# Lzcstan/DrugLAMP

Hardware: AMD Instinct MI355X
Metric: drug-protein pairs/sec training step (higher is better)
Workload: dtype bf16; 1 GPU; DrugLAMP training step (cls step, epoch 1; fwd+bwd+grad all-reduce+AdamW), BindingDB-shaped synthetic pairs (512 drug nodes/tokens, 2304 protein tokens = 256 sites, pre-extracted 384-d/640-d LLM embeddings), global batch 256 = 256 per GPU x 1; per_gpu_batch=256, global_batch=256, parallelism=dp1, step_kind=cls, epoch=1, hip_graph=False, protein_seq_len=2304, distinct_batches=8, first_touch_steps=8, padding_rows=computed once, protein_cnn_rows=distinct rows, streams=independent branches on side HIP streams

## Files before the change

druglamp_amd/_lib.py:

```python
from __future__ import annotations

import ctypes as C
import os

import torch

_HERE = os.path.dirname(os.path.abspath(__file__))
_variant = os.environ.get("DL_USE_STUDY_LIB", "")
if _variant and not _variant.endswith(".so"):
    raise RuntimeError("DL_USE_STUDY_LIB=%s: the -DDL_STUDY build (libdruglamp_hip_study.so) was removed; commit 97fb613 is the last "
                       "that builds it (python -m druglamp_amd.build --study).  Only a variant library name (libdruglamp_hip_<variant>.so) "
                       "is accepted." % _variant)
LIB_PATH = os.path.join(_HERE, "lib", _variant or "libdruglamp_hip.so")

DL_F32, DL_BF16 = 0, 1

c_i64, c_i32, c_f32, c_u64, c_vp, c_sz = C.c_int64, C.c_int32, C.c_float, C.c_uint64, C.c_void_p, C.c_size_t


class ReduceItem(C.Structure):
    _fields_ = [
        ("kind", c_i32), ("out_dtype", c_i32),
        ("src", c_vp), ("out", c_vp),
        ("mn", c_i64), ("ldc", c_i64),
        ("N", c_i32), ("splits", c_i32), ("accumulate", c_i32), ("M", c_i32),
        ("cs_slabs", c_vp), ("cs_out", c_vp),
    ]


REDUCE_BATCH_MAX = 24
GEMM_GROUP_MAX = 16


class GemmArgs(C.Structure):
    _fields_ = [
        ("X", c_vp), ("ldx", c_i64), ("x_kslow", c_i32),
        ("W", c_vp), ("ldw", c_i64), ("w_kslow", c_i32),
        ("C", c_vp), ("ldc", c_i64),
        ("M", c_i64), ("N", c_i64), ("K", c_i64),
        ("in_dtype", c_i32), ("out_dtype", c_i32),
        ("bias", c_vp),
        ("residual", c_vp), ("ldr", c_i64),
        ("res_row_mod", c_i64),
        ("res_before_dropout", c_i32),
        ("act", c_i32),
        ("pre_out", c_vp), ("ldp", c_i64),
        ("dact_pre", c_vp), ("lddp", c_i64),
        ("dropout_p", c_f32), ("dropout_seed", c_u64),
        ("accumulate", c_i32),
        ("split_k", c_i32), ("workspace", c_vp), ("workspace_bytes", c_sz),
        ("x_colsum", c_vp),
        ("dropout_seed_offset", c_vp),
        ("algo", c_i32),
        ("tile_tickets", c_vp),
        ("deferred", C.POINTER(ReduceItem)),
        ("prof_tag", c_i32),
    ]


FLAG_PROT_PERIOD, FLAG_DRUG_TOKEN_PAD, FLAG_GCN_NODE_PAD, FLAG_PLAN_ROWS, FLAG_PAIR_INDEX = 1, 2, 4, 8, 16
FLAG_KEY_TABLE = 32
FLAG_MAP_COLS = 64
TAG_OTHER, TAG_QKV_OUT, TAG_FFN, TAG_CONV, TAG_WGRAD, TAG_ADAPTOR = 0, 1, 2, 3, 4, 5
TAG_NAMES = {0: "other", 1: "qkv_out", 2: "ffn", 3: "conv", 4: "wgrad", 5: "adaptor"}


class AttnFwdArgs(C.Structure):
    _fields_ = [
        ("Q", c_vp), ("K", c_vp), ("V", c_vp), ("O", c_vp), ("LSE", c_vp), ("raw_logits", c_vp),
        ("q_ps", c_i64), ("q_hs", c_i64), ("q_rs", c_i64),
        ("k_ps", c_i64), ("k_hs", c_i64), ("k_rs", c_i64),
        ("v_ps", c_i64), ("v_hs", c_i64), ("v_rs", c_i64),
        ("o_ps", c_i64), ("o_hs", c_i64), ("o_rs", c_i64), ("o_ss", c_i64),
        ("n_problems", c_i32), ("n_heads", c_i32), ("n_segments", c_i32), ("partner_shift", c_i32),
        ("Lq", c_i32), ("Lk", c_i32), ("head_dim", c_i32), ("dtype", c_i32),
        ("scale", c_f32),
        ("algo", c_i32),
        ("key_tail_rows", c_i32), ("key_tail_weight", c_f32),
    ]


class AttnBwdArgs(C.Structure):
    _fields_ = [
        ("Q", c_vp), ("K", c_vp), ("V", c_vp), ("O", c_vp), ("dO", c_vp),
        ("LSE", c_vp), ("Delta", c_vp),
        ("dQ", c_vp), ("dK", c_vp), ("dV", c_vp),
        ("q_ps", c_i64), ("q_hs", c_i64), ("q_rs", c_i64),
        ("k_ps", c_i64), ("k_hs", c_i64), ("k_rs", c_i64),
        ("v_ps", c_i64), ("v_hs", c_i64), ("v_rs", c_i64),
        ("o_ps", c_i64), ("o_hs", c_i64), ("o_rs", c_i64), ("o_ss", c_i64),
        ("do_ps", c_i64), ("do_hs", c_i64), ("do_rs", c_i64), ("do_ss", c_i64),
        ("dq_ps", c_i64), ("dq_hs", c_i64), ("dq_rs", c_i64),
        ("dk_ps", c_i64), ("dk_hs", c_i64), ("dk_rs", c_i64),
        ("dv_ps", c_i64), ("dv_hs", c_i64), ("dv_rs", c_i64),
        ("n_problems", c_i32), ("n_heads", c_i32), ("n_segments", c_i32), ("partner_shift", c_i32),
        ("Lq", c_i32), ("Lk", c_i32), ("head_dim", c_i32), ("dtype", c_i32),
        ("scale", c_f32),
        ("algo", c_i32),
        ("key_tail_rows", c_i32), ("key_tail_weight", c_f32),
    ]


class AttnProbsArgs(C.Structure):
    _fields_ = [
        ("Q", c_vp), ("K", c_vp), ("LSE", c_vp), ("out", c_vp), ("out_ld", c_i64),
        ("q_ps", c_i64), ("q_hs", c_i64), ("q_rs", c_i64),
        ("k_ps", c_i64), ("k_hs", c_i64), ("k_rs", c_i64),
        ("n_problems", c_i32), ("n_heads", c_i32), ("n_segments", c_i32), ("partner_shift", c_i32),
        ("Lq", c_i32), ("Lk", c_i32), ("head_dim", c_i32), ("dtype", c_i32),
        ("scale", c_f32),
        ("head_mean", c_i32), ("key_tail_rows", c_i32), ("key_tail_weight", c_f32), ("expand_tail", c_i32),
        ("workspace", c_vp), ("workspace_bytes", c_sz),
    ]


# ... 66 lines not shown
        ("q_index", c_vp), ("kv_index", c_vp), ("kv_row0", c_vp), ("kv_keys", c_vp), ("kv_tail_weight", c_vp), ("flags", c_vp),
        ("q_es", c_i64), ("q_rs", c_i64), ("k_rs", c_i64), ("mass_ps", c_i64), ("site_ps", c_i64), ("kv_total_rows", c_i64),
        ("n_pairs", c_i32), ("n_q", c_i32), ("n_kv", c_i32), ("Lq", c_i32), ("head_dim", c_i32), ("dtype", c_i32),
        ("out_cols", c_i32),
        ("scale", c_f32),
        ("key_tail_rows", c_i32),
        ("reserved", c_i32),
    ]


class PgcaPairsAttrArgs(C.Structure):
    _fields_ = [
        ("Q", c_vp), ("K", c_vp), ("dO", c_vp), ("sites", c_vp), ("d_sites", c_vp), ("key_attr", c_vp), ("site_attr", c_vp),
        ("q_index", c_vp), ("kv_index", c_vp), ("flags", c_vp),
        ("q_es", c_i64), ("q_rs", c_i64), ("k_es", c_i64), ("k_rs", c_i64), ("do_ps", c_i64), ("do_rs", c_i64),
        ("left_es", c_i64), ("left_rs", c_i64), ("dl_ps", c_i64), ("dl_rs", c_i64), ("mass_ps", c_i64), ("site_ps", c_i64),
        ("n_pairs", c_i32), ("n_q", c_i32), ("n_kv", c_i32), ("Lq", c_i32), ("Lk", c_i32), ("head_dim", c_i32), ("dtype", c_i32),
        ("out_cols", c_i32), ("left_cols", c_i32),
        ("scale", c_f32),
        ("key_tail_rows", c_i32), ("key_tail_weight", c_f32),
        ("reserved", c_i32),
    ]


class PgcaPairsRaggedAttrArgs(C.Structure):
    _fields_ = [
        ("Q", c_vp), ("K", c_vp), ("dO", c_vp), ("sites", c_vp), ("d_sites", c_vp), ("key_attr", c_vp), ("site_attr", c_vp),
        ("q_index", c_vp), ("kv_index", c_vp), ("kv_row0", c_vp), ("kv_keys", c_vp), ("kv_tail_weight", c_vp), ("flags", c_vp),
        ("q_es", c_i64), ("q_rs", c_i64), ("k_rs", c_i64), ("do_ps", c_i64), ("do_rs", c_i64),
        ("left_es", c_i64), ("left_rs", c_i64), ("dl_ps", c_i64), ("dl_rs", c_i64), ("mass_ps", c_i64), ("site_ps", c_i64),
        ("kv_total_rows", c_i64),
        ("n_pairs", c_i32), ("n_q", c_i32), ("n_kv", c_i32), ("Lq", c_i32), ("head_dim", c_i32), ("dtype", c_i32),
        ("out_cols", c_i32), ("left_cols", c_i32),
        ("scale", c_f32),
        ("key_tail_rows", c_i32),
        ("reserved", c_i32),
    ]


class NtxentSide(C.Structure):
    _fields_ = [("q", c_vp), ("k", c_vp), ("n", c_i64), ("gid_offset", c_i64), ("lse", c_vp)]


class NtxentArgs(C.Structure):
    _fields_ = [("a", NtxentSide), ("b", NtxentSide), ("n_global", c_i64), ("d", c_i64), ("dtype", c_i32),
                ("temperature", c_f32)]


SIGNATURES = {
    "dl_last_error": (C.c_char_p, []),
    "dl_version": (c_i32, []),
    "dl_gemm_workspace_bytes": (c_sz, [C.POINTER(GemmArgs)]),
    "dl_gemm": (c_i32, [C.POINTER(GemmArgs), c_vp]),
    "dl_gemm_pair": (c_i32, [C.POINTER(GemmArgs), C.POINTER(GemmArgs), c_vp]),
    "dl_gemm_group_plan": (c_i32, [C.POINTER(GemmArgs), c_i32, C.POINTER(c_i32)]),
    "dl_gemm_group": (c_i32, [C.POINTER(GemmArgs), c_i32, c_vp]),
    "dl_reduce_batch": (c_i32, [C.POINTER(ReduceItem), c_i32, c_vp]),
    "dl_colsum": (c_i32, [c_vp, c_i64, c_i64, c_i64, c_i32, c_vp, c_i32, c_vp, c_sz, c_vp]),
    "dl_colsum_workspace_bytes": (c_sz, [c_i64, c_i64]),
    "dl_bn_workspace_bytes": (c_sz, [c_i64, c_i64]),
    "dl_bn_stats": (c_i32, [c_vp, c_i64, c_i64, c_i64, c_i64, c_i64, c_i32, c_vp, c_vp, c_sz, c_vp]),
    "dl_bn_apply_fwd": (c_i32, [c_vp, c_vp, c_vp, c_vp, c_vp, c_vp, c_i64, c_i64, c_i64, c_i64, c_i64, c_i32, c_vp]),
    "dl_bn_bwd_reduce": (c_i32, [c_vp, c_vp, c_vp, c_vp, c_i64, c_i64, c_i64, c_i64, c_i64, c_i32, c_vp, c_vp, c_sz, c_vp]),
    "dl_bn_tail_fix": (c_i32, [c_vp, c_vp, c_vp, c_vp, c_vp, c_vp, c_f32, c_i32, c_i64, c_i64, c_i64, c_i64, c_i32, c_vp]),
    "dl_bn_apply_relu_fwd": (c_i32, [c_vp, c_vp, c_vp, c_vp, c_vp, c_vp, c_i64, c_i64, c_i32, c_vp]),
    "dl_bn_relu_bwd": (c_i32, [c_vp, c_vp, c_vp, c_vp, c_vp, c_vp, c_f32, c_vp, c_vp, c_i64, c_i64, c_i32, c_vp, c_sz, c_vp]),
    "dl_bn_bwd_apply": (c_i32, [c_vp, c_vp, c_vp, c_vp, c_vp, c_vp, c_f32, c_i32, c_vp, c_i64, c_i64, c_i64, c_i64, c_i64,
                                c_i32, c_vp]),
    "dl_layernorm_fwd": (c_i32, [c_vp, c_i64, c_vp, c_vp, c_vp, c_i64, c_vp, c_vp, c_i64, c_i64, c_f32, c_i32, c_vp]),
    "dl_layernorm_bwd_workspace_bytes": (c_sz, [c_i64, c_i64]),
    "dl_layernorm_bwd": (c_i32, [c_vp, c_i64, c_i64, c_vp, c_i64, c_vp, c_vp, c_vp, c_vp, c_i64, c_vp, c_i64, c_vp, c_vp,
                                 c_i32, c_i64, c_i64, c_i32, c_vp, c_sz, C.POINTER(ReduceItem), c_vp]),
    "dl_attn_fwd": (c_i32, [C.POINTER(AttnFwdArgs), c_vp]),
    "dl_attn_bwd": (c_i32, [C.POINTER(AttnBwdArgs), c_vp]),
    "dl_attn_probs_workspace_bytes": (c_sz, [C.POINTER(AttnProbsArgs)]),
    "dl_attn_probs": (c_i32, [C.POINTER(AttnProbsArgs), c_vp]),
    "dl_pgca_pairs_fwd": (c_i32, [C.POINTER(PgcaPairsArgs), c_vp]),
    "dl_pgca_pairs_ragged_fwd": (c_i32, [C.POINTER(PgcaPairsRaggedArgs), c_vp]),
    "dl_pgca_pairs_probs": (c_i32, [C.POINTER(PgcaPairsProbsArgs), c_vp]),
    "dl_pgca_pairs_ragged_probs": (c_i32, [C.POINTER(PgcaPairsRaggedProbsArgs), c_vp]),
    "dl_pgca_pairs_profile": (c_i32, [C.POINTER(PgcaPairsProfileArgs), c_vp]),
    "dl_pgca_pairs_ragged_profile": (c_i32, [C.POINTER(PgcaPairsRaggedProfileArgs), c_vp]),
    "dl_pgca_pairs_attr": (c_i32, [C.POINTER(PgcaPairsAttrArgs), c_vp]),
    "dl_pgca_pairs_ragged_attr": (c_i32, [C.POINTER(PgcaPairsRaggedAttrArgs), c_vp]),
    "dl_token_gate_fwd": (c_i32, [c_vp, c_vp, c_vp, c_vp, c_i64, c_i64, c_i64, c_i32, c_i32, c_i32, c_vp]),
    "dl_token_gate_bwd": (c_i32, [c_vp, c_vp, c_vp, c_vp, c_vp, c_i64, c_i64, c_i64, c_i32, c_i32, c_i32, c_vp]),
    "dl_gate_dpre": (c_i32, [c_vp, c_vp, c_vp, c_vp, c_i64, c_i64, c_i32, c_i32, c_vp]),
    "dl_add_rowmod_dropout": (c_i32, [c_vp, c_vp, c_vp, c_i64, c_i64, c_i64, c_f32, c_u64, c_vp, c_i32, c_vp]),
    "dl_dropout_apply": (c_i32, [c_vp, c_vp, c_i64, c_i64, c_i64, c_i64, c_f32, c_u64, c_vp, c_i32, c_vp]),
    "dl_fill_pool": (c_i32, [c_vp, c_vp, c_vp, c_i64, c_i64, c_i64, c_i32, c_i32, c_i32, c_vp]),
    "dl_cnn_sitepool_fwd": (c_i32, [c_vp, c_vp, c_i64, c_i64, c_i64, c_i32, c_i32, c_i32, c_vp]),
    "dl_cnn_sitepool_bwd": (c_i32, [c_vp, c_vp, c_i64, c_i64, c_i64, c_i32, c_i32, c_i32, c_vp]),
    "dl_bn_stats_finalize": (c_i32, [c_vp, c_i64, c_i64, c_i64, c_i64, c_i64, c_vp, c_i32, c_i64, c_f32, c_f32, c_vp, c_vp, c_vp, c_vp, c_vp, c_vp, c_vp, c_sz, c_vp]),
    "dl_bn_finalize": (c_i32, [c_vp, c_i64, c_f32, c_f32, c_vp, c_vp, c_vp, c_vp, c_vp, c_i64, c_vp]),
    "dl_interleave_streams": (c_i32, [c_vp, c_vp, c_i64, c_i64, c_i32, c_i32, c_vp]),
    "dl_norm_adjacency": (c_i32, [c_vp, c_vp, c_i64, c_i32, c_i32, c_vp]),
    "dl_graph_aggregate": (c_i32, [c_vp, c_vp, c_vp, c_i64, c_i32, c_i32, c_i32, c_i32, c_i32, c_vp]),
    "dl_concat2": (c_i32, [c_vp, c_vp, c_vp, c_i64, c_i64, c_i64, c_i32, c_vp]),
    "dl_gather_pad": (c_i32, [c_vp, c_vp, c_vp, c_vp, c_i64, c_i64, c_i64, c_i32, c_i32, c_vp]),
    "dl_embed_pad": (c_i32, [c_vp, c_vp, c_vp, c_vp, c_i64, c_i64, c_i32, c_i32, c_i32, c_i32, c_vp]),
    "dl_weight_prep": (c_i32, [c_vp, c_vp, c_i32, c_i32, c_vp]),
    "dl_gelu_bwd": (c_i32, [c_vp, c_vp, c_vp, c_i64, c_i32, c_vp]),
    "dl_cast": (c_i32, [c_vp, c_i32, c_vp, c_i32, c_i64, c_vp]),
    "dl_rowmod_sum": (c_i32, [c_vp, c_vp, c_i64, c_i64, c_i64, c_i32, c_i32, c_vp]),
    "dl_cos_rowloss_fwd": (c_i32, [c_vp, c_vp, c_vp, c_vp, c_i64, c_i64, c_vp]),
    "dl_cos_rowloss_bwd": (c_i32, [c_vp, c_vp, c_f32, c_vp, c_i64, c_i64, c_vp]),
# ... 128 lines not shown
```

druglamp_amd/csrc/gemm.hip:

```cpp
#include <stdlib.h>
#include <stdint.h>
#include <algorithm>
#include <type_traits>
#include "common.cuh"

namespace {

constexpr int BKB = 128;
constexpr int NTHREADS = 256;

template <typename T, int TW> struct TileGeom {
  static constexpr int BT = 32 * TW;
  static constexpr int BKE = BKB / (int)sizeof(T);
  static constexpr int PITCH_KSLOW = BT * (int)sizeof(T);
  static constexpr int CPR_KSLOW = PITCH_KSLOW / 16;
  static constexpr int TILE_KCONTIG = BT * BKB;
  static constexpr int TILE_KSLOW = BKE * PITCH_KSLOW;
  static constexpr int TILE_BYTES = TILE_KSLOW > TILE_KCONTIG ? TILE_KSLOW : TILE_KCONTIG;
};

struct GemmP {
  const char* X; const char* W; char* C;
  int64_t ldx, ldw, ldc;
  int M, N, K, k_per_split, mt, nt, splits;
// ... 372 lines not shown
        if (full) {
          const f32x4 q0 = load4<T>(src), q1 = load4<T>(src + 4);
#pragma unroll
          for (int r = 0; r < 4; ++r) { resv[r] = q0[r]; resv[4 + r] = q1[r]; }
        } else {
          for (int r = 0; r < nvalid; ++r) resv[r] = to_f32(src[r]);
        }
        if (p.res_before_dropout) {
#pragma unroll
          for (int r = 0; r < 8; ++r) v[r] += resv[r];
        }
      }
      if (p.drop_thr16) {
        f32x4 d0 = {v[0], v[1], v[2], v[3]}, d1 = {v[4], v[5], v[6], v[7]};
        d0 = dl_dropout4(d0, p.seed + seed_off_v, (uint64_t)m, (uint64_t)n, (uint64_t)p.N, p.drop_thr16, p.drop_inv_keep);
        d1 = dl_dropout4(d1, p.seed + seed_off_v, (uint64_t)m, (uint64_t)(n + 4), (uint64_t)p.N, p.drop_thr16, p.drop_inv_keep);
#pragma unroll
        for (int r = 0; r < 4; ++r) { v[r] = d0[r]; v[4 + r] = d1[r]; }
      }
      if (p.res && !p.res_before_dropout) {
#pragma unroll
        for (int r = 0; r < 8; ++r) v[r] += resv[r];
      }
      TO* dst = reinterpret_cast<TO*>(p.C) + (int64_t)m * p.ldc + n;
      if (p.accumulate) {
        if (full) {
          const f32x4 o0 = load4<TO>(dst), o1 = load4<TO>(dst + 4);
#pragma unroll
          for (int r = 0; r < 4; ++r) { v[r] += o0[r]; v[4 + r] += o1[r]; }
        } else {
          for (int r = 0; r < nvalid; ++r) v[r] += to_f32(dst[r]);
        }
      }
      if (full) {
        if constexpr (sizeof(TO) == 2) {
          u32x4 o = {pack_bf16x2(v[0], v[1]), pack_bf16x2(v[2], v[3]), pack_bf16x2(v[4], v[5]), pack_bf16x2(v[6], v[7])};
          *reinterpret_cast<u32x4*>(dst) = o;
        } else {
          *reinterpret_cast<f32x4*>(dst) = f32x4{v[0], v[1], v[2], v[3]};
          *reinterpret_cast<f32x4*>(dst + 4) = f32x4{v[4], v[5], v[6], v[7]};
        }
      } else {
        for (int r = 0; r < nvalid; ++r) dst[r] = from_f32<TO>(v[r]);
      }
    }
  }
  if (!have_next) break;
  it = itn;
  __syncthreads();
  }
}

#include "gemm_big.cuh"

template <typename TO>
__global__ void splitk_reduce_kernel(const float* __restrict__ slabs, TO* __restrict__ out,
                                     int64_t mn, int64_t ldc, int N, int splits, int accumulate,
                                     const float* __restrict__ cs_slabs, float* __restrict__ cs_out, int M, uint32_t main_blocks) {
  if (blockIdx.x >= main_blocks) {
    const int m = (int)(blockIdx.x - main_blocks) * blockDim.x + threadIdx.x;
    if (m < M) {
      float a0 = 0.f, a1 = 0.f;
      int z = 0;
      for (; z + 1 < splits; z += 2) { a0 += cs_slabs[(int64_t)z * M + m]; a1 += cs_slabs[(int64_t)(z + 1) * M + m]; }
      if (z < splits) a0 += cs_slabs[(int64_t)z * M + m];
      cs_out[m] = a0 + a1;
    }
    return;
  }
  const int64_t i4 = ((int64_t)blockIdx.x * blockDim.x + threadIdx.x) * 4;
  if (i4 >= mn) return;
  f32x4 s0 = {0.f, 0.f, 0.f, 0.f}, s1 = s0, s2 = s0, s3 = s0;
  int z = 0;
  for (; z + 3 < splits; z += 4) {
    s0 += *reinterpret_cast<const f32x4*>(slabs + (int64_t)z * mn + i4);
    s1 += *reinterpret_cast<const f32x4*>(slabs + (int64_t)(z + 1) * mn + i4);
    s2 += *reinterpret_cast<const f32x4*>(slabs + (int64_t)(z + 2) * mn + i4);
    s3 += *reinterpret_cast<const f32x4*>(slabs + (int64_t)(z + 3) * mn + i4);
  }
  for (; z < splits; ++z) s0 += *reinterpret_cast<const f32x4*>(slabs + (int64_t)z * mn + i4);
  f32x4 s = (s0 + s1) + (s2 + s3);
  const int64_t m = i4 / N, n = i4 % N;
  TO* dst = out + m * ldc + n;
  if (accumulate) { const f32x4 o = load4<TO>(dst); s += o; }
  store4<TO>(dst, s);
}

int pick_tw(const dl_gemm_args* a) {
  if (a->x_kslow && a->w_kslow && a->split_k >= 0) {
    const int64_t tiles128 = ((a->M + 127) / 128) * ((a->N + 127) / 128);
    if (tiles128 <= 4 && a->M >= 64 && a->N >= 64 && a->K % (BKB / (int)dl_dtype_size(a->in_dtype)) == 0) return 2;
  }
  return 4;
}

int auto_split(int64_t M, int64_t N, int64_t K, int bke, int bt) {
  const int64_t tiles = ((M + bt - 1) / bt) * ((N + bt - 1) / bt);
  if (tiles >= 192) return 1;
  constexpr int round_wgs = 512, max_sp = 256;
  int64_t want = round_wgs / tiles;
  if (want < 1) want = 1;
  int64_t ksteps = (K + bke - 1) / bke;
  int64_t maxs = ksteps / 4;
  if (maxs < 1) maxs = 1;
  if (want > maxs) want = maxs;
  if (want > max_sp) want = max_sp;
  return (int)(want < 1 ? 1 : want);
}

int big_tt_plan(const dl_gemm_args* a, int* bm_out);
static int trim_splits(int64_t K, int step, int sp) {
  const int64_t ksteps = (K + step - 1) / step;
  if (sp > ksteps) sp = (int)ksteps;
  if (sp < 1) sp = 1;
  const int64_t per = (ksteps + sp - 1) / sp;
  return (int)((ksteps + per - 1) / per);
}
int resolve_split(const dl_gemm_args* a) {
  { const int sp = big_tt_plan(a, nullptr); if (sp > 0) return trim_splits(a->K, 64, sp); }
  const int bke = BKB / (int)dl_dtype_size(a->in_dtype);
  if (a->split_k > 0) return trim_splits(a->K, bke, a->split_k);
  if (a->split_k < 0) return 1;
  const bool plain = !a->bias && !a->residual && !a->act && !a->pre_out && !a->dact_pre &&
                     a->dropout_p <= 0.f && a->out_dtype == DL_F32 && (a->N % 4 == 0);
  return plain ? trim_splits(a->K, bke, auto_split(a->M, a->N, a->K, bke, 32 * pick_tw(a))) : 1;
}

int pick_epi(const GemmP& p, bool split) {
  int epi = 1;
  if (!split && (p.N % 8 == 0) && !p.accumulate && p.res_row_mod == 0 && !(p.res && p.res_before_dropout)) {
    const bool drop = p.drop_thr16 != 0;
    if (!p.res && !p.act && !p.pre_out && !p.dact_pre && !drop) epi = 0;
    else if (p.act == 1 && p.pre_out && !p.res && !p.dact_pre) epi = 2;
    else if (p.res && !p.act && !p.pre_out && !p.dact_pre) epi = 3;
    else if (p.dact_pre && !p.res && !p.act && !p.pre_out && !p.bias) epi = 4;
    else if (p.act == 2 && !p.res && !p.pre_out && !p.dact_pre && !drop) epi = 5;
  }
  return epi;
}

bool big_eligible(const dl_gemm_args* a, const GemmP& p, int sp) {
  if (a->algo == DL_GEMM_ALGO_TILE128) return false;
  if (sp > 1 || a->in_dtype != DL_BF16 || a->out_dtype != DL_BF16 || a->x_kslow || a->w_kslow) return false;
  if (pick_epi(p, false) == 1) return false;
  if (a->K % 64 != 0 || a->N <= 128) return false;
  const int64_t tiles = ((a->M + 255) / 256) * ((a->N + 255) / 256);
  return tiles >= 192;
}
constexpr int LAT_MIN_K = 512;
constexpr int LAT_MAX_TILES = 256;
bool lat_eligible(const dl_gemm_args* a, const GemmP& p, int sp) {
  if (a->algo == DL_GEMM_ALGO_TILE128) return false;
  if (sp > 1 || a->in_dtype != DL_BF16 || a->out_dtype != DL_BF16 || a->x_kslow || a->w_kslow) return false;
  if (pick_epi(p, false) == 1) return false;
  if (a->K % 64 != 0 || a->K < LAT_MIN_K || a->N < 128) return false;
  const int64_t tiles = ((a->M + 127) / 128) * ((a->N + 127) / 128);
  return tiles <= LAT_MAX_TILES;
}
template <int XF, int WM, int WN, int RB, int NS>
void launch_big_form(const GemmP& p, hipStream_t s, uint32_t max_wgs, uint32_t threads) {
  const uint32_t ntiles = (uint32_t)p.mt * p.nt;
  const uint32_t nblocks = ntiles < max_wgs ? ntiles : max_wgs;
#define DL_BIG(E) hipLaunchKernelGGL((gemm_big_kernel<XF, WM, WN, RB, NS, E>), dim3(nblocks), dim3(threads), 0, s, p)
  switch (pick_epi(p, false)) {
    case 0: DL_BIG(0); break;
    case 2: DL_BIG(2); break;
    case 3: DL_BIG(3); break;
    case 4: DL_BIG(4); break;
    default: DL_BIG(5); break;
  }
#undef DL_BIG
}
void launch_lat(const GemmP& p, hipStream_t s) { launch_big_form<4, 2, 2, 128, 4>(p, s, 256u, 256u); }
void launch_big(const GemmP& p, hipStream_t s) { launch_big_form<8, 2, 4, 128, 2>(p, s, 256u, 512u); }

int big_tt_plan(const dl_gemm_args* a, int* bm_out) {
  if (a->algo == DL_GEMM_ALGO_TILE128) return 0;
  if (a->in_dtype != DL_BF16 || !a->x_kslow || !a->w_kslow || a->split_k != 0) return 0;
  const bool plain = !a->bias && !a->residual && !a->act && !a->pre_out && !a->dact_pre && a->dropout_p <= 0.f;
  if (!plain || a->M % 8 != 0 || a->N % 8 != 0 || a->N < 192 || a->M < 96 || a->K < 4096) return 0;
  const bool big = a->M > 128 && a->M * a->N >= 640 * 1024;
  const int bm = big ? 256 : 128;
  if (!big) {
    const double work = (double)a->M * (double)a->N * (double)a->K;
    if (a->M > 128 ? work < 1.0e10 : (a->N < 640 || a->K < 262144)) return 0;
  }
  const int64_t tiles = ((a->M + bm - 1) / bm) * ((a->N + 255) / 256);
  if (tiles > 256) return 0;
  int64_t sp = 256 / tiles;
  const int64_t ksteps = (a->K + 63) / 64;
  if (sp > ksteps / 4) sp = ksteps / 4;
  if (sp < 1) sp = 1;
  if (bm_out) *bm_out = bm;
  return (int)sp;
}
template <int XF, int KS, int NS, bool PF>
void launch_big_tt2(const GemmP& p, hipStream_t s, uint32_t nblocks) {
  if (p.cs_slabs) hipLaunchKernelGGL((gemm_big_tt2_kernel<XF, 2, 4, true, KS, NS, PF>), dim3(nblocks), dim3(512), 0, s, p);
  else hipLaunchKernelGGL((gemm_big_tt2_kernel<XF, 2, 4, false, KS, NS, PF>), dim3(nblocks), dim3(512), 0, s, p);
}
void launch_big_tt(const GemmP& p, hipStream_t s, int bm) {
  const uint32_t ntiles = (uint32_t)p.mt * p.nt * p.splits;
  const uint32_t nblocks = ntiles < 256u ? ntiles : 256u;
  if (bm == 256) launch_big_tt2<8, 32, 4, false>(p, s, nblocks); else launch_big_tt2<4, 64, 3, false>(p, s, nblocks);
}

template <typename T, typename TO, bool XS, bool WS, bool SPLIT, bool DMA>
void launch(const GemmP& p, hipStream_t s, int tw) {
  const int epi = pick_epi(p, SPLIT);
  const uint32_t ntiles = (uint32_t)p.mt * p.nt * p.splits;
// ... 20 lines not shown
      case 2: DL_LAUNCH(2); break;
      case 3: DL_LAUNCH(3); break;
      case 4: DL_LAUNCH(4); break;
      case 5: DL_LAUNCH(5); break;
      default: DL_LAUNCH(1); break;
    }
  }
#undef DL_LAUNCH
}

template <typename T, typename TO, bool SPLIT>
int dispatch_layout(const dl_gemm_args* a, const GemmP& p, hipStream_t s, int tw) {
  const int bke = BKB / (int)sizeof(T);
  const bool dma = (a->K % bke == 0) && (p.k_per_split % bke == 0);
  if (!a->x_kslow && !a->w_kslow) { if (dma) launch<T, TO, false, false, SPLIT, true>(p, s, tw); else launch<T, TO, false, false, SPLIT, false>(p, s, tw); }
  else if (!a->x_kslow && a->w_kslow) { if (dma) launch<T, TO, false, true, SPLIT, true>(p, s, tw); else launch<T, TO, false, true, SPLIT, false>(p, s, tw); }
  else if (a->x_kslow && a->w_kslow) { if (dma) launch<T, TO, true, true, SPLIT, true>(p, s, tw); else launch<T, TO, true, true, SPLIT, false>(p, s, tw); }
  else {
    dl_set_error("dl_gemm: layout x_kslow=1,w_kslow=0 is not instantiated");
    return DL_ERR_UNSUPPORTED;
  }
  return DL_OK;
}

}

extern "C" size_t dl_gemm_workspace_bytes(const dl_gemm_args* a) {
  if (!a) return 0;
  const int sp = resolve_split(a);
  const size_t cs = a->x_colsum ? (size_t)sp * (size_t)a->M * sizeof(float) : 0;
  if (big_tt_plan(a, nullptr) > 0 || sp > 1 || a->x_colsum) return (size_t)sp * (size_t)a->M * (size_t)a->N * sizeof(float) + cs;
  return 0;
}

namespace {
static double gemm_algorithmic_bytes(const dl_gemm_args* a) {
  const double es = (double)dl_dtype_size(a->in_dtype), oes = (double)dl_dtype_size(a->out_dtype);
  auto span = [](double rows, double len, double pitch) { return pitch < len ? (rows - 1.0) * pitch + len : rows * len; };
  const double x = a->x_kslow ? span((double)a->K, (double)a->M, (double)a->ldx) : span((double)a->M, (double)a->K, (double)a->ldx);
  const double w = a->w_kslow ? span((double)a->K, (double)a->N, (double)a->ldw) : span((double)a->N, (double)a->K, (double)a->ldw);
  const double mn = (double)a->M * (double)a->N;
  double bytes = (x + w) * es + mn * oes;
  if (a->pre_out) bytes += mn * es;
  if (a->dact_pre) bytes += mn * es;
  if (a->residual) bytes += (a->res_row_mod > 0 ? (double)a->res_row_mod * (double)a->N : mn) * es;
  if (a->accumulate) bytes += mn * oes;
  if (a->bias) bytes += (double)a->N * 4.0;
  return bytes;
}
constexpr int DL_PAIR_FALLBACK = 1;
int gemm_run(const dl_gemm_args* a, const dl_gemm_args* b, dl_stream stream);
}
extern "C" int dl_gemm(const dl_gemm_args* a, dl_stream stream) { return gemm_run(a, nullptr, stream); }

extern "C" int dl_gemm_pair(const dl_gemm_args* a, const dl_gemm_args* b, dl_stream stream) {
  DL_CHECK_ARG(a && b, DL_ERR_ARG, "dl_gemm_pair: null argument block");
  auto same_presence = [](const void* x, const void* y) { return (x == nullptr) == (y == nullptr); };
  const bool twin =
      a->M == b->M && a->N == b->N && a->K == b->K && a->ldx == b->ldx && a->ldw == b->ldw && a->ldc == b->ldc &&
      a->x_kslow == b->x_kslow && a->w_kslow == b->w_kslow && a->in_dtype == b->in_dtype && a->out_dtype == b->out_dtype &&
      a->ldr == b->ldr && a->res_row_mod == b->res_row_mod && a->res_before_dropout == b->res_before_dropout &&
      a->act == b->act && a->ldp == b->ldp && a->lddp == b->lddp && a->dropout_p == b->dropout_p &&
      a->accumulate == b->accumulate && a->split_k == b->split_k && a->algo == b->algo &&
      a->dropout_seed_offset == b->dropout_seed_offset && a->tile_tickets == b->tile_tickets &&
      same_presence(a->bias, b->bias) && same_presence(a->residual, b->residual) && same_presence(a->pre_out, b->pre_out) &&
      same_presence(a->dact_pre, b->dact_pre) && !a->x_colsum && !b->x_colsum && !a->deferred && !b->deferred &&
      (((uintptr_t)b->X | (uintptr_t)b->W | (uintptr_t)b->C | (uintptr_t)b->bias | (uintptr_t)b->residual |
        (uintptr_t)b->pre_out | (uintptr_t)b->dact_pre) & 15) == 0;
  if (twin) {
    const int rc = gemm_run(a, b, stream);
    if (rc != DL_PAIR_FALLBACK) return rc;
  }
  const int rc = gemm_run(a, nullptr, stream);
  return rc != DL_OK ? rc : gemm_run(b, nullptr, stream);
}

namespace {
int gemm_run(const dl_gemm_args* a, const dl_gemm_args* b, dl_stream stream) {
  hipStream_t s = (hipStream_t)stream;
  DL_CHECK_ARG(a && a->X && a->W && a->C, DL_ERR_ARG, "dl_gemm: null operand");
  if (b) DL_CHECK_ARG(b->X && b->W && b->C, DL_ERR_ARG, "dl_gemm_pair: null operand");
  DL_CHECK_ARG(a->M > 0 && a->N > 0 && a->K > 0, DL_ERR_SHAPE, "dl_gemm: bad shape M=%ld N=%ld K=%ld",
               (long)a->M, (long)a->N, (long)a->K);
  DL_CHECK_ARG(a->M < (1ll << 30) && a->N < (1ll << 30) && a->K < (1ll << 30), DL_ERR_SHAPE,
               "dl_gemm: dims must fit int32");
  DL_CHECK_ARG(a->in_dtype == DL_F32 || a->in_dtype == DL_BF16, DL_ERR_ARG, "dl_gemm: bad in_dtype");
  DL_CHECK_ARG(a->out_dtype == DL_F32 || a->out_dtype == a->in_dtype, DL_ERR_ARG,
               "dl_gemm: out_dtype must be f32 or in_dtype");
  const int es = (int)dl_dtype_size(a->in_dtype);
  const int epc = 16 / es;
  DL_CHECK_ARG(a->ldx % epc == 0 && a->ldw % epc == 0, DL_ERR_ALIGN,
               "dl_gemm: ldx/ldw must be multiples of %d elements", epc);
  DL_CHECK_ARG(((uintptr_t)a->X & 15) == 0 && ((uintptr_t)a->W & 15) == 0, DL_ERR_ALIGN,
               "dl_gemm: X/W must be 16-byte aligned");
  if (!a->x_kslow) DL_CHECK_ARG(a->K % epc == 0, DL_ERR_ALIGN, "dl_gemm: K %% %d != 0", epc);
  else DL_CHECK_ARG(a->M % epc == 0, DL_ERR_ALIGN, "dl_gemm: M %% %d != 0 for k-slow X", epc);
  if (!a->w_kslow) DL_CHECK_ARG(a->K % epc == 0, DL_ERR_ALIGN, "dl_gemm: K %% %d != 0", epc);
  else DL_CHECK_ARG(a->N % epc == 0, DL_ERR_ALIGN, "dl_gemm: N %% %d != 0 for k-slow W", epc);
  if (a->N % 8 == 0) {
    DL_CHECK_ARG(a->ldc % 8 == 0 && ((uintptr_t)a->C % 16) == 0, DL_ERR_ALIGN,
                 "dl_gemm: C / ldc not aligned for 16-byte stores (N %% 8 == 0 path)");
    DL_CHECK_ARG(!a->residual || (a->ldr % 8 == 0 && ((uintptr_t)a->residual % 16) == 0), DL_ERR_ALIGN,
                 "dl_gemm: residual not 16-byte aligned");
    DL_CHECK_ARG(!a->pre_out || (a->ldp % 8 == 0 && ((uintptr_t)a->pre_out % 16) == 0), DL_ERR_ALIGN,
                 "dl_gemm: pre_out not 16-byte aligned");
    DL_CHECK_ARG(!a->dact_pre || (a->lddp % 8 == 0 && ((uintptr_t)a->dact_pre % 16) == 0), DL_ERR_ALIGN,
                 "dl_gemm: dact_pre not 16-byte aligned");
    DL_CHECK_ARG(!a->bias || ((uintptr_t)a->bias % 16) == 0, DL_ERR_ALIGN, "dl_gemm: bias not 16-byte aligned");
  }
  DL_CHECK_ARG(a->dropout_p >= 0.f && a->dropout_p < 1.f, DL_ERR_ARG, "dl_gemm: dropout_p out of range");
  DL_CHECK_ARG(a->dropout_p == 0.f || a->N % 8 == 0, DL_ERR_SHAPE, "dl_gemm: dropout needs N %% 8 == 0");
  DL_CHECK_ARG(a->algo == DL_GEMM_ALGO_AUTO || a->algo == DL_GEMM_ALGO_TILE128, DL_ERR_ARG, "dl_gemm: bad algo %d", a->algo);

  const int sp = resolve_split(a);
  int tt_bm = 0;
  const bool big_tt = big_tt_plan(a, &tt_bm) > 0;
  if (a->x_colsum)
    DL_CHECK_ARG(a->x_kslow && a->w_kslow && a->split_k == 0, DL_ERR_UNSUPPORTED,
                 "dl_gemm: x_colsum needs the weight-gradient form (x_kslow, w_kslow, split_k = 0)");
  const bool slab_path = sp > 1 || big_tt || a->x_colsum != nullptr;
  if (slab_path) {
    DL_CHECK_ARG(!a->bias && !a->residual && !a->act && !a->pre_out && !a->dact_pre &&
                     a->dropout_p == 0.f && (a->N % 4 == 0),
                 DL_ERR_UNSUPPORTED, "dl_gemm: split_k supports only the plain epilogue, N %% 4 == 0");
    const size_t need = dl_gemm_workspace_bytes(a);
    DL_CHECK_ARG(a->workspace && a->workspace_bytes >= need, DL_ERR_WORKSPACE,
                 "dl_gemm: split_k=%d needs %zu workspace bytes, got %zu", sp, need, a->workspace_bytes);
  }

  GemmP p;
  p.X = (const char*)a->X; p.W = (const char*)a->W; p.C = (char*)a->C;
  p.ldx = a->ldx; p.ldw = a->ldw; p.ldc = a->ldc;
  p.M = (int)a->M; p.N = (int)a->N; p.K = (int)a->K;
  const int tw = slab_path ? pick_tw(a) : 4;
  const int bt = 32 * tw;
  p.mt = (int)((a->M + bt - 1) / bt); p.nt = (int)((a->N + bt - 1) / bt); p.splits = sp;
  const int bke = BKB / es;
  {
    const int64_t ksteps = (a->K + bke - 1) / bke;
    const int64_t per = (ksteps + sp - 1) / sp;
    p.k_per_split = (int)(per * bke);
  }
  p.bias = a->bias;
  p.res = (const char*)a->residual; p.ldr = a->ldr; p.res_row_mod = (int)a->res_row_mod;
  p.res_before_dropout = a->res_before_dropout;
  p.act = a->act;
  p.pre_out = (char*)a->pre_out; p.ldp = a->ldp;
  p.dact_pre = (const char*)a->dact_pre; p.lddp = a->lddp;
  p.drop_thr16 = a->dropout_p > 0.f ? dl_dropout_thr16(a->dropout_p) : 0u;
  p.drop_inv_keep = a->dropout_p > 0.f ? 1.0f / (1.0f - a->dropout_p) : 1.0f;
  p.seed = a->dropout_seed; p.seed_off = a->dropout_seed_offset;
  p.tickets = a->tile_tickets;
  p.accumulate = a->accumulate;
  p.slabs = (float*)a->workspace;
  p.cs_slabs = a->x_colsum ? (float*)a->workspace + (size_t)sp * a->M * a->N : nullptr;
  p.nt_c = 1; p.nt_pre = 1; p.nt_small = 1;
  p.nt_ext = 0;

  if (b) {
    if (slab_path || big_eligible(a, p, sp) || lat_eligible(a, p, sp)) return DL_PAIR_FALLBACK;
    p.nprob = 2;
    p.dX = (const char*)b->X - (const char*)a->X; p.dW = (const char*)b->W - (const char*)a->W;
    p.dC = (char*)b->C - (char*)a->C;
    p.dBias = a->bias ? (const char*)b->bias - (const char*)a->bias : 0;
    p.dRes = a->residual ? (const char*)b->residual - (const char*)a->residual : 0;
    p.dPre = a->pre_out ? (char*)b->pre_out - (char*)a->pre_out : 0;
    p.dDact = a->dact_pre ? (const char*)b->dact_pre - (const char*)a->dact_pre : 0;
    p.dSeed = b->dropout_seed - a->dropout_seed;
  }
  dl_prof_before(0, s);
  int rc = DL_OK;
  if (big_tt) {
    p.mt = (int)((a->M + tt_bm - 1) / tt_bm); p.nt = (int)((a->N + 255) / 256);
    const int64_t ksteps = (a->K + 63) / 64;
    p.k_per_split = (int)(((ksteps + sp - 1) / sp) * 64);
    launch_big_tt(p, s, tt_bm);
  } else if (big_eligible(a, p, sp)) {
    p.mt = (int)((a->M + 255) / 256); p.nt = (int)((a->N + 255) / 256);
    launch_big(p, s);
  } else if (!b && lat_eligible(a, p, sp)) {
    p.mt = (int)((a->M + 127) / 128); p.nt = (int)((a->N + 127) / 128);
    launch_lat(p, s);
  } else if (a->in_dtype == DL_BF16) {
    if (slab_path) rc = dispatch_layout<bf16_t, float, true>(a, p, s, tw);
    else if (a->out_dtype == DL_F32) rc = dispatch_layout<bf16_t, float, false>(a, p, s, tw);
    else rc = dispatch_layout<bf16_t, bf16_t, false>(a, p, s, tw);
  } else {
    if (slab_path) rc = dispatch_layout<float, float, true>(a, p, s, tw);
    else rc = dispatch_layout<float, float, false>(a, p, s, tw);
  }
  if (rc != DL_OK) return rc;
  DL_CHECK_LAUNCH("dl_gemm");
  {
    const double flops = 2.0 * (double)a->M * (double)a->N * (double)a->K * (b ? 2 : 1);
    dl_prof_after(0, s, flops, gemm_algorithmic_bytes(a) * (b ? 2 : 1), a->prof_tag);
  }
  if (slab_path) {
    const int64_t mn = a->M * a->N;
    if (a->deferred) {
      dl_reduce_item& it = *a->deferred;
      it.kind = DL_REDUCE_SPLITK; it.out_dtype = a->out_dtype;
      it.src = (const float*)a->workspace; it.out = a->C; it.mn = mn; it.ldc = a->ldc; it.N = (int32_t)a->N;
      it.splits = sp; it.accumulate = a->accumulate; it.M = a->x_colsum ? (int32_t)a->M : 0;
      it.cs_slabs = p.cs_slabs; it.cs_out = a->x_colsum;
      return DL_OK;
    }
    const int threads = 256;
    const int64_t blocks = (mn / 4 + threads - 1) / threads;
    const int64_t cs_blocks = a->x_colsum ? (a->M + threads - 1) / threads : 0;
    if (a->out_dtype == DL_F32)
      hipLaunchKernelGGL((splitk_reduce_kernel<float>), dim3((uint32_t)(blocks + cs_blocks)), dim3(threads), 0, s,
                         (const float*)a->workspace, (float*)a->C, mn, a->ldc, (int)a->N, sp,
                         a->accumulate, (const float*)p.cs_slabs, a->x_colsum, (int)a->M, (uint32_t)blocks);
    else
      hipLaunchKernelGGL((splitk_reduce_kernel<bf16_t>), dim3((uint32_t)(blocks + cs_blocks)), dim3(threads), 0, s,
                         (const float*)a->workspace, (bf16_t*)a->C, mn, a->ldc, (int)a->N, sp,
                         a->accumulate, (const float*)p.cs_slabs, a->x_colsum, (int)a->M, (uint32_t)blocks);
    DL_CHECK_LAUNCH("dl_gemm(split reduce)");
  } else if (a->deferred) {
    a->deferred->kind = DL_REDUCE_NONE;
  }
  return DL_OK;
}
}

namespace {
bool group_member_ok(const dl_gemm_args* a) {
  const bool plain = !a->bias && !a->residual && !a->act && !a->pre_out && !a->dact_pre && a->dropout_p <= 0.f && !a->accumulate;
  return a->X && a->W && a->C && a->in_dtype == DL_BF16 && a->out_dtype == DL_F32 && a->x_kslow && a->w_kslow && a->split_k == 0 && plain &&
         a->algo == DL_GEMM_ALGO_AUTO && a->M >= 8 && a->N >= 8 && a->M % 8 == 0 && a->N % 8 == 0 && a->K >= 64 &&
         a->M < (1ll << 30) && a->N < (1ll << 30) && a->K < (1ll << 30) && a->ldx % 8 == 0 && a->ldw % 8 == 0 &&
         (((uintptr_t)a->X | (uintptr_t)a->W | (uintptr_t)a->C) & 15) == 0 && a->ldc % 4 == 0;
}
int group_plan(const dl_gemm_args* args, int n, int* splits, int* bm_out) {
  if (!args || n < 1 || n > DL_GROUP_MAX) return 0;
// ... 156 lines not shown
```

include/druglamp_hip.h:

```cpp
#ifndef DRUGLAMP_HIP_H
#define DRUGLAMP_HIP_H

#include <stddef.h>
#include <stdint.h>

#ifdef __cplusplus
extern "C" {
#endif

typedef enum { DL_OK = 0, DL_ERR_ARG = -1, DL_ERR_SHAPE = -2, DL_ERR_ALIGN = -3,
               DL_ERR_WORKSPACE = -4, DL_ERR_LAUNCH = -5, DL_ERR_UNSUPPORTED = -6 } dl_status;

typedef enum { DL_F32 = 0, DL_BF16 = 1 } dl_dtype;

typedef void* dl_stream;

const char* dl_last_error(void);
int dl_version(void);

typedef struct dl_reduce_item {
  int32_t kind;
  int32_t out_dtype;
  const float* src;
  void* out;
  int64_t mn;
  int64_t ldc;
  int32_t N;
  int32_t splits;
  int32_t accumulate;
  int32_t M;
  const float* cs_slabs;
  float* cs_out;
} dl_reduce_item;
enum { DL_REDUCE_NONE = 0, DL_REDUCE_SPLITK = 1, DL_REDUCE_PARTIALS = 2 };
enum { DL_REDUCE_BATCH_MAX = 24 };
int dl_reduce_batch(const dl_reduce_item* items, int32_t n, dl_stream s);

typedef struct {
  const void* X; int64_t ldx; int32_t x_kslow;
  const void* W; int64_t ldw; int32_t w_kslow;
  void* C; int64_t ldc;
  int64_t M, N, K;
  int32_t in_dtype, out_dtype;
  const float* bias;
  const void* residual; int64_t ldr;
  int64_t res_row_mod;
  int32_t res_before_dropout;
  int32_t act;
  void* pre_out; int64_t ldp;
  const void* dact_pre; int64_t lddp;
  float dropout_p; uint64_t dropout_seed;
  int32_t accumulate;
  int32_t split_k; void* workspace; size_t workspace_bytes;
  float* x_colsum;
  const uint64_t* dropout_seed_offset;
  int32_t algo;
  int32_t* tile_tickets;
  dl_reduce_item* deferred;
  int32_t prof_tag;
} dl_gemm_args;
enum { DL_TAG_OTHER = 0, DL_TAG_QKV_OUT = 1, DL_TAG_FFN = 2, DL_TAG_CONV = 3, DL_TAG_WGRAD = 4, DL_TAG_ADAPTOR = 5 };
enum { DL_GEMM_ALGO_AUTO = 0, DL_GEMM_ALGO_TILE128 = 1 };

size_t dl_gemm_workspace_bytes(const dl_gemm_args* a);
int dl_gemm(const dl_gemm_args* a, dl_stream s);
int dl_gemm_pair(const dl_gemm_args* a, const dl_gemm_args* b, dl_stream s);
int dl_gemm_group_plan(const dl_gemm_args* args, int32_t n, int32_t* splits_out);
int dl_gemm_group(const dl_gemm_args* args, int32_t n, dl_stream s);

int dl_colsum(const void* X, int64_t ldx, int64_t M, int64_t N, int32_t dtype, float* out,
              int32_t accumulate, void* workspace, size_t workspace_bytes, dl_stream s);
size_t dl_colsum_workspace_bytes(int64_t M, int64_t N);

size_t dl_bn_workspace_bytes(int64_t R, int64_t C);
int dl_bn_stats(const void* y, int64_t R, int64_t C, int64_t win, int64_t halo, int64_t valid,
                int32_t dtype, float* sums, void* workspace, size_t workspace_bytes, dl_stream s);
int dl_bn_finalize(const float* sums, int64_t n, float eps, float momentum, float* mean, float* var, float* rstd,
                   float* running_mean, float* running_var, int64_t C, dl_stream s);
int dl_bn_apply_fwd(const void* y, void* z, const float* mean, const float* rstd, const float* gamma,
                    const float* beta, int64_t R, int64_t C, int64_t win, int64_t halo, int64_t valid,
                    int32_t dtype, dl_stream s);
int dl_bn_bwd_reduce(const void* dz, const void* y, const float* mean, const float* rstd, int64_t R,
                     int64_t C, int64_t win, int64_t halo, int64_t valid, int32_t dtype, float* sums,
                     void* workspace, size_t workspace_bytes, dl_stream s);
int dl_bn_bwd_apply(const void* dz, const void* y, const float* mean, const float* rstd,
                    const float* gamma, const float* sums, float inv_n, int32_t relu_mask, void* dy,
                    int64_t R, int64_t C, int64_t win, int64_t halo, int64_t valid, int32_t dtype,
                    dl_stream s);
int dl_bn_stats_rw(const void* y, int64_t R, int64_t C, const float* row_w, int32_t dtype, float* sums, void* workspace,
                   size_t workspace_bytes, dl_stream s);
int dl_bn_stats_finalize(const void* y, int64_t R, int64_t C, int64_t win, int64_t halo, int64_t valid, const float* row_w,
                         int32_t dtype, int64_t n, float eps, float momentum, float* sums, float* mean, float* var, float* rstd,
                         float* running_mean, float* running_var, void* workspace, size_t workspace_bytes, dl_stream s);
int dl_bn_apply_fwd_rw(const void* y, void* z, const float* mean, const float* rstd, const float* gamma, const float* beta,
                       int64_t R, int64_t C, const float* row_w, int32_t dtype, dl_stream s);
int dl_bn_bwd_reduce_rw(const void* dz, const void* y, const float* mean, const float* rstd, int64_t R, int64_t C,
                        const float* row_w, int32_t dtype, float* sums, void* workspace, size_t workspace_bytes, dl_stream s);
int dl_bn_bwd_apply_rw(const void* dz, const void* y, const float* mean, const float* rstd, const float* gamma,
                       const float* sums, float inv_n, int32_t relu_mask, void* dy, int64_t R, int64_t C, const float* row_w,
                       int32_t dtype, dl_stream s);
int dl_bn_tail_fix(void* dy, const void* y, const float* mean, const float* rstd, const float* gamma, const float* sums,
                   float inv_n, int32_t w, int64_t R, int64_t C, int64_t win, int64_t lead, int32_t dtype, dl_stream s);
int dl_bn_apply_relu_fwd(const void* y, void* z, const float* mean, const float* rstd, const float* gamma, const float* beta,
                         int64_t R, int64_t C, int32_t dtype, dl_stream s);
int dl_bn_relu_bwd(const void* dz, const void* y, const float* mean, const float* rstd, const float* gamma, const float* beta,
                   float inv_n, void* dy, float* sums, int64_t R, int64_t C, int32_t dtype, void* workspace, size_t workspace_bytes,
                   dl_stream s);
int dl_bn_eval_bwd(const void* dz, const void* y, const float* mean, const float* rstd, const float* gamma, const float* beta,
                   int32_t relu_in, int32_t relu_out, void* dy, float* sums, int64_t R, int64_t C, int64_t win, int64_t halo,
                   int64_t valid, const float* row_w, int32_t dtype, void* workspace, size_t workspace_bytes, dl_stream s);

int dl_layernorm_fwd(const void* x, int64_t ldx, const float* gamma, const float* beta, void* y,
                     int64_t ldy, float* mean, float* rstd, int64_t M, int64_t D, float eps,
                     int32_t dtype, dl_stream s);
size_t dl_layernorm_bwd_workspace_bytes(int64_t M, int64_t D);
// ... 269 lines not shown
```

Baseline: 20730 pairs/s.

## Add warp-specialized streaming GEMM kernel for tall-skinny bf16 GEMMs

Adds a new GEMM path for bf16 problems with small N (at most 128) and small K (at most 256). The kernel keeps the whole weight matrix resident in LDS and streams 32-row X blocks through a multi-stage ring. Four producer waves issue direct-to-LDS loads while four consumer waves run MFMA, with a fused bias/ReLU epilogue. It is auto-selected whenever M is at least 32 and the other paths don't apply, which targets adaptor and projection GEMMs over many rows. A path-query API is also added. The risk is worse tile efficiency or occupancy than the existing tile128 path for some shapes.

```diff
diff --git a/druglamp_amd/_lib.py b/druglamp_amd/_lib.py
--- a/druglamp_amd/_lib.py
+++ b/druglamp_amd/_lib.py
@@ -61,6 +61,8 @@
 FLAG_PROT_PERIOD, FLAG_DRUG_TOKEN_PAD, FLAG_GCN_NODE_PAD, FLAG_PLAN_ROWS, FLAG_PAIR_INDEX = 1, 2, 4, 8, 16
 FLAG_KEY_TABLE = 32
 FLAG_MAP_COLS = 64
+GEMM_ALGO_AUTO, GEMM_ALGO_TILE128, GEMM_ALGO_STREAM = 0, 1, 2
+GEMM_PATH_TILE128, GEMM_PATH_BIG256, GEMM_PATH_LAT128, GEMM_PATH_TT2, GEMM_PATH_STREAM = 0, 1, 2, 3, 4
 TAG_OTHER, TAG_QKV_OUT, TAG_FFN, TAG_CONV, TAG_WGRAD, TAG_ADAPTOR = 0, 1, 2, 3, 4, 5
 TAG_NAMES = {0: "other", 1: "qkv_out", 2: "ffn", 3: "conv", 4: "wgrad", 5: "adaptor"}
 
@@ -233,6 +235,8 @@
     "dl_version": (c_i32, []),
     "dl_gemm_workspace_bytes": (c_sz, [C.POINTER(GemmArgs)]),
     "dl_gemm": (c_i32, [C.POINTER(GemmArgs), c_vp]),
+    "dl_gemm_path": (c_i32, [C.POINTER(GemmArgs)]),
+    "dl_gemm_stream_min_m": (c_i64, []),
     "dl_gemm_pair": (c_i32, [C.POINTER(GemmArgs), C.POINTER(GemmArgs), c_vp]),
     "dl_gemm_group_plan": (c_i32, [C.POINTER(GemmArgs), c_i32, C.POINTER(c_i32)]),
     "dl_gemm_group": (c_i32, [C.POINTER(GemmArgs), c_i32, c_vp]),
diff --git a/druglamp_amd/csrc/gemm.hip b/druglamp_amd/csrc/gemm.hip
--- a/druglamp_amd/csrc/gemm.hip
+++ b/druglamp_amd/csrc/gemm.hip
@@ -448,6 +448,7 @@
 }
 
 #include "gemm_big.cuh"
+#include "gemm_stream.cuh"
 
 template <typename TO>
 __global__ void splitk_reduce_kernel(const float* __restrict__ slabs, TO* __restrict__ out,
@@ -552,6 +553,33 @@
   if (a->K % 64 != 0 || a->K < LAT_MIN_K || a->N < 128) return false;
   const int64_t tiles = ((a->M + 127) / 128) * ((a->N + 127) / 128);
   return tiles <= LAT_MAX_TILES;
+}
+constexpr int64_t STREAM_MIN_M = 32;
+constexpr uint32_t STREAM_MAX_WGS = 256;
+bool stream_eligible(const dl_gemm_args* a, const GemmP& p, int sp) {
+  if (a->algo == DL_GEMM_ALGO_TILE128) return false;
+  if (sp > 1 || a->in_dtype != DL_BF16 || a->out_dtype != DL_BF16 || a->x_kslow || a->w_kslow) return false;
+  const int epi = pick_epi(p, false);
+  if (epi != 0 && epi != 5) return false;
+  if (a->N > 128 || a->N % 16 != 0 || a->K % 64 != 0 || a->K > 256) return false;
+  if (a->ldx < a->K || a->ldw < a->K || a->ldc < a->N) return false;
+  return a->algo == DL_GEMM_ALGO_STREAM || a->M >= STREAM_MIN_M;
+}
+template <int EPI>
+void launch_stream_epi(const GemmP& p, hipStream_t s) {
+  const uint32_t nblk = (uint32_t)((p.M + STREAM_BM - 1) / STREAM_BM);
+  const uint32_t nblocks = nblk < STREAM_MAX_WGS ? nblk : STREAM_MAX_WGS;
+#define DL_STREAM(KS) hipLaunchKernelGGL((gemm_stream_kernel<KS, EPI>), dim3(nblocks), dim3(512), 0, s, p)
+  switch (p.K / 64) {
+    case 1: DL_STREAM(1); break;
+    case 2: DL_STREAM(2); break;
+    case 3: DL_STREAM(3); break;
+    default: DL_STREAM(4); break;
+  }
+#undef DL_STREAM
+}
+void launch_stream(const GemmP& p, hipStream_t s) {
+  if (pick_epi(p, false) == 5) launch_stream_epi<5>(p, s); else launch_stream_epi<0>(p, s);
 }
 template <int XF, int WM, int WN, int RB, int NS>
 void launch_big_form(const GemmP& p, hipStream_t s, uint32_t max_wgs, uint32_t threads) {
@@ -678,6 +706,21 @@
 int gemm_run(const dl_gemm_args* a, const dl_gemm_args* b, dl_stream stream);
 }
 extern "C" int dl_gemm(const dl_gemm_args* a, dl_stream stream) { return gemm_run(a, nullptr, stream); }
+
+extern "C" int32_t dl_gemm_path(const dl_gemm_args* a) {
+  if (!a) return -1;
+  GemmP p;
+  p.N = (int)a->N; p.bias = a->bias; p.res = (const char*)a->residual; p.res_row_mod = (int)a->res_row_mod;
+  p.res_before_dropout = a->res_before_dropout; p.act = a->act; p.pre_out = (char*)a->pre_out;
+  p.dact_pre = (const char*)a->dact_pre; p.drop_thr16 = a->dropout_p > 0.f ? 1u : 0u; p.accumulate = a->accumulate;
+  const int sp = resolve_split(a);
+  if (big_tt_plan(a, nullptr) > 0) return DL_GEMM_PATH_TT2;
+  if (big_eligible(a, p, sp)) return DL_GEMM_PATH_BIG256;
+  if (lat_eligible(a, p, sp)) return DL_GEMM_PATH_LAT128;
+  if (sp == 1 && !a->x_colsum && stream_eligible(a, p, sp)) return DL_GEMM_PATH_STREAM;
+  return DL_GEMM_PATH_TILE128;
+}
+extern "C" int64_t dl_gemm_stream_min_m(void) { return STREAM_MIN_M; }
 
 extern "C" int dl_gemm_pair(const dl_gemm_args* a, const dl_gemm_args* b, dl_stream stream) {
   DL_CHECK_ARG(a && b, DL_ERR_ARG, "dl_gemm_pair: null argument block");
@@ -736,7 +779,7 @@
   }
   DL_CHECK_ARG(a->dropout_p >= 0.f && a->dropout_p < 1.f, DL_ERR_ARG, "dl_gemm: dropout_p out of range");
   DL_CHECK_ARG(a->dropout_p == 0.f || a->N % 8 == 0, DL_ERR_SHAPE, "dl_gemm: dropout needs N %% 8 == 0");
-  DL_CHECK_ARG(a->algo == DL_GEMM_ALGO_AUTO || a->algo == DL_GEMM_ALGO_TILE128, DL_ERR_ARG, "dl_gemm: bad algo %d", a->algo);
+  DL_CHECK_ARG(a->algo == DL_GEMM_ALGO_AUTO || a->algo == DL_GEMM_ALGO_TILE128 || a->algo == DL_GEMM_ALGO_STREAM, DL_ERR_ARG, "dl_gemm: bad algo %d", a->algo);
 
   const int sp = resolve_split(a);
   int tt_bm = 0;
@@ -807,6 +850,8 @@
   } else if (!b && lat_eligible(a, p, sp)) {
     p.mt = (int)((a->M + 127) / 128); p.nt = (int)((a->N + 127) / 128);
     launch_lat(p, s);
+  } else if (!b && stream_eligible(a, p, sp)) {
+    launch_stream(p, s);
   } else if (a->in_dtype == DL_BF16) {
     if (slab_path) rc = dispatch_layout<bf16_t, float, true>(a, p, s, tw);
     else if (a->out_dtype == DL_F32) rc = dispatch_layout<bf16_t, float, false>(a, p, s, tw);
diff --git a/druglamp_amd/csrc/gemm_stream.cuh b/druglamp_amd/csrc/gemm_stream.cuh
--- /dev/null
+++ b/druglamp_amd/csrc/gemm_stream.cuh
@@ -0,0 +1,133 @@
+#pragma once
+
+template <int N> __device__ __forceinline__ void stream_wait_blocks(int blocks) {
+  switch (blocks) {
+    case 0: wait_vmcnt<0>(); break;
+    case 1: wait_vmcnt<N>(); break;
+    case 2: wait_vmcnt<2 * N>(); break;
+    case 3: wait_vmcnt<3 * N>(); break;
+    case 4: wait_vmcnt<4 * N>(); break;
+    case 5: wait_vmcnt<5 * N>(); break;
+    default: wait_vmcnt<6 * N>(); break;
+  }
+}
+
+constexpr int STREAM_BM = 32;
+constexpr int stream_nst(int ks) { return ks >= 4 ? 5 : (ks == 3 ? 6 : 8); }
+
+template <int KS, int EPI>
+__global__ __launch_bounds__(512, 2) void gemm_stream_kernel(const GemmP p) {
+  typedef bf16_t T;
+  constexpr int BM = STREAM_BM, NST = stream_nst(KS);
+  constexpr int WSLAB = 128 * 128, XSLAB = BM * 128;
+  constexpr int WB = KS * WSLAB, STAGE = KS * XSLAB;
+  static_assert(NST >= 3 && NST <= 8 && (NST - 2) * KS < 64, "ring depth / vmcnt immediate");
+  static_assert(WB + NST * STAGE <= 160 * 1024, "LDS");
+  __shared__ __attribute__((aligned(16))) char smem[WB + NST * STAGE];
+
+  const int tid = threadIdx.x, lane = tid & 63;
+  const int wave = __builtin_amdgcn_readfirstlane(tid >> 6);
+
+  const uint32_t nblk = (uint32_t)((p.M + BM - 1) / BM), G = gridDim.x, b = blockIdx.x;
+  const uint32_t q = nblk / G, r = nblk % G;
+  const uint32_t first = b * q + (b < r ? b : r);
+  const int nb = (int)(q + (b < r ? 1u : 0u));
+  if (nb == 0) return;
+
+  if (wave >= 4) {
+    const int lw = wave - 4, ltid = lw * 64 + lane;
+    const uint32_t smem_lds = (uint32_t)(size_t)(__attribute__((address_space(3))) char*)smem;
+    const int drow = ltid >> 3, dkc = ((ltid & 7) ^ (drow & 7)) * 16;
+    auto issue_x = [&](int blk, int stage) {
+      int gr = (int)(first + (uint32_t)blk) * BM + drow;
+      gr = gr < p.M ? gr : p.M - 1;
+      const char* src = p.X + (int64_t)gr * p.ldx * 2 + dkc;
+      const uint32_t dst = smem_lds + (uint32_t)(WB + stage * STAGE + lw * 1024);
+#pragma unroll
+      for (int ks = 0; ks < KS; ++ks) dma16(src + ks * 128, __builtin_amdgcn_readfirstlane(dst + (uint32_t)(ks * XSLAB)));
+    };
+#pragma unroll
+    for (int ks = 0; ks < KS; ++ks)
+#pragma unroll
+      for (int i = 0; i < 4; ++i) {
+        int wr = drow + i * 32;
+        wr = wr < p.N ? wr : p.N - 1;
+        dma16(p.W + (int64_t)wr * p.ldw * 2 + dkc + ks * 128,
+              __builtin_amdgcn_readfirstlane(smem_lds + (uint32_t)(ks * WSLAB + (i * 256 + lw * 64) * 16)));
+      }
+#pragma unroll
+    for (int s = 0; s < NST - 1; ++s)
+      if (s < nb) issue_x(s, s);
+    int stage = 0;
+    for (int i = 0; i < nb; ++i) {
+      stream_wait_blocks<KS>(min(NST - 2, nb - 1 - i));
+      wg_barrier();
+      if (i + NST - 1 < nb) issue_x(i + NST - 1, stage == 0 ? NST - 1 : stage - 1);
+      stage = stage + 1 == NST ? 0 : stage + 1;
+    }
+    return;
+  }
+
+  const int il = lane & 15, g = lane >> 4;
+  f32x4 bj[2];
+#pragma unroll
+  for (int j = 0; j < 2; ++j) {
+    const int n = wave * 32 + j * 16 + 4 * g;
+    bj[j] = f32x4{0.f, 0.f, 0.f, 0.f};
+    if (p.bias != nullptr && n < p.N) bj[j] = *reinterpret_cast<const f32x4*>(p.bias + n);
+  }
+  asm volatile("" : "+v"(bj[0]), "+v"(bj[1]));
+
+  const int xoff = il * 128, woff = (wave * 32 + il) * 128, swz = il & 7;
+  int stage = 0;
+  for (int i = 0; i < nb; ++i) {
+    asm volatile("s_waitcnt lgkmcnt(0)" ::: "memory");
+    wg_barrier();
+    const char* xs = smem + WB + stage * STAGE;
+    f32x4 acc[2][2];
+#pragma unroll
+    for (int a = 0; a < 2; ++a)
+#pragma unroll
+      for (int j = 0; j < 2; ++j) acc[a][j] = f32x4{0.f, 0.f, 0.f, 0.f};
+#pragma unroll
+    for (int ks = 0; ks < KS; ++ks)
+#pragma unroll
+      for (int kf = 0; kf < 2; ++kf) {
+        const uint32_t ch = (uint32_t)(((kf * 4 + g) ^ swz) << 4);
+        u32x4 fx[2], fw[2];
+#pragma unroll
+        for (int a = 0; a < 2; ++a) fx[a] = lds_read16(xs, ks * XSLAB + xoff + a * 16 * 128 + ch);
+#pragma unroll
+        for (int j = 0; j < 2; ++j) fw[j] = lds_read16(smem, ks * WSLAB + woff + j * 16 * 128 + ch);
+#pragma unroll
+        for (int a = 0; a < 2; ++a)
+#pragma unroll
+          for (int j = 0; j < 2; ++j) acc[a][j] = Mma<T>::mma(fw[j], fx[a], acc[a][j]);
+      }
+    const int m0 = (int)(first + (uint32_t)i) * BM;
+    const int ncol = wave * 32 + (g & 1) * 16 + (g >> 1) * 8;
+#pragma unroll
+    for (int a = 0; a < 2; ++a) {
+      uint32_t pk[2][2];
+#pragma unroll
+      for (int j = 0; j < 2; ++j) {
+        f32x4 v = acc[a][j];
+        v += bj[j];
+        if constexpr (EPI == 5) {
+#pragma unroll
+          for (int e = 0; e < 4; ++e) v[e] = max_keep_nan(v[e], 0.f);
+        }
+        pk[j][0] = pack_bf16x2(v[0], v[1]); pk[j][1] = pack_bf16x2(v[2], v[3]);
+      }
+      const bool odd = (g & 1) != 0;
+      const uint32_t s0 = odd ? pk[0][0] : pk[1][0], s1 = odd ? pk[0][1] : pk[1][1];
+      const uint32_t r0 = (uint32_t)__shfl_xor((int)s0, 16), r1 = (uint32_t)__shfl_xor((int)s1, 16);
+      const u32x4 o = odd ? u32x4{r0, r1, pk[1][0], pk[1][1]} : u32x4{pk[0][0], pk[0][1], r0, r1};
+      const int m = m0 + a * 16 + il;
+      if (m < p.M && ncol < p.N) {
+        *reinterpret_cast<u32x4*>(p.C + ((int64_t)m * p.ldc + ncol) * 2) = o;
+      }
+    }
+    stage = stage + 1 == NST ? 0 : stage + 1;
+  }
+}
diff --git a/include/druglamp_hip.h b/include/druglamp_hip.h
--- a/include/druglamp_hip.h
+++ b/include/druglamp_hip.h
@@ -60,7 +60,10 @@
   int32_t prof_tag;
 } dl_gemm_args;
 enum { DL_TAG_OTHER = 0, DL_TAG_QKV_OUT = 1, DL_TAG_FFN = 2, DL_TAG_CONV = 3, DL_TAG_WGRAD = 4, DL_TAG_ADAPTOR = 5 };
-enum { DL_GEMM_ALGO_AUTO = 0, DL_GEMM_ALGO_TILE128 = 1 };
+enum { DL_GEMM_ALGO_AUTO = 0, DL_GEMM_ALGO_TILE128 = 1, DL_GEMM_ALGO_STREAM = 2 };
+enum { DL_GEMM_PATH_TILE128 = 0, DL_GEMM_PATH_BIG256 = 1, DL_GEMM_PATH_LAT128 = 2, DL_GEMM_PATH_TT2 = 3, DL_GEMM_PATH_STREAM = 4 };
+int32_t dl_gemm_path(const dl_gemm_args* a);
+int64_t dl_gemm_stream_min_m(void);
 
 size_t dl_gemm_workspace_bytes(const dl_gemm_args* a);
 int dl_gemm(const dl_gemm_args* a, dl_stream s);
```

After: 20700 pairs/s. No clear change (-0.2%).
